# MILVLG/mmnas

Hardware: AMD Instinct MI355X
Metric: supernet fwd+bwd steps/sec (VQA arch, bs=64) (higher is better)
Workload: dtype f32 (bf16x6 split-operand MFMA, fp32 accumulate); 1 GPU; Net_Search supernet WEIGHT step: sample + fwd + BCE(sum) + bwd (+ gradient all-reduce), HSIZE 256, B=64/GPU, 100x2048 regions + 14 tokens, dropout 0.1 (search_vqa.py:279-292; BASELINE configs[2]); global_batch=64, parallelism=dp1, grad_allreduce=none, rccl_ranks=1, rank_id_sum_ok=True, lstm_fallback=False, dp_rows=1, dp_buckets=3, optimizer_in_step=False, gemm_split=6, hip_force_dev_kernarg=1

## Files before the change

### include/mmnas_hip.h

```cpp
#ifndef MMNAS_HIP_H
#define MMNAS_HIP_H

#include <stddef.h>
#include <stdint.h>

#ifdef __cplusplus
extern "C" {
#endif

#define MMNAS_ABI_VERSION 1

enum {
  MMNAS_OK = 0,
  MMNAS_E_SHAPE = -1,
  MMNAS_E_ARG = -2,
  MMNAS_E_LAUNCH = -3
};

enum {
  MMNAS_F_NORM = 1,
  MMNAS_F_RESIDUAL = 2,
  MMNAS_F_MASK = 4,
  MMNAS_F_REL = 8,
  MMNAS_F_SELF = 16,
// ... 146 lines not shown
int mmnas_rel_fused_bwd(const float* raw, const float* Wy, const float* by, const float* Wr,
                        const float* br, const float* dbiasT, float* dWy, float* dby, float* dWr,
                        float* dbr, float* ws, int B, int Sq, int Sk, int C, int R, int H,
                        void* stream);
int mmnas_rel_fused_fwd_ragged(const float* raw, const float* Wy, const float* by, const float* Wr, const float* br,
                               float* biasT, int B, int S, int C, int R, int H, const int* off, void* stream);
int mmnas_rel_fused_bwd_ragged(const float* raw, const float* Wy, const float* by, const float* Wr, const float* br,
                               const float* dbiasT, float* dWy, float* dby, float* dWr, float* dbr, float* ws,
                               int B, int S, int C, int R, int H, const int* off, const int* tile_off, int ntiles, void* stream);

#define MMNAS_REL_MULTI_MAX 32
typedef struct mmnas_rel_multi {
  int B, S, C, R, H, n_ops;
  const float* raw;
  const float* Wy; const float* by;
  float* dWy; float* dby;
  const float* Wr[MMNAS_REL_MULTI_MAX];
  const float* br[MMNAS_REL_MULTI_MAX];
  float* biasT[MMNAS_REL_MULTI_MAX];
  const float* dbiasT[MMNAS_REL_MULTI_MAX];
  float* dWr[MMNAS_REL_MULTI_MAX]; float* dbr[MMNAS_REL_MULTI_MAX];
  const int* off; const int* tile_off; int ntiles, reserved;
  float* ws;
} mmnas_rel_multi;
int mmnas_rel_multi_supported(int C, int R, int H);
size_t mmnas_rel_multi_bwd_ws_floats(int B, int S);
int mmnas_rel_multi_fwd(const mmnas_rel_multi* m, void* stream);
int mmnas_rel_multi_bwd(const mmnas_rel_multi* m, void* stream);
int mmnas_set_rel_hoist(int on);
int mmnas_set_guided_hoist(int on);
int mmnas_set_rel_overlap(int on);

typedef struct mmnas_mha_desc {
  int B, H, Sq, Sk, dh;
  int ldq, ldk, ldv, ldo;
  const float* Q; const float* K; const float* V;
  const uint8_t* mask;
  const float* biasT;
  float* O;
  float* lse;
  float drop_p; uint32_t drop_site; uint64_t drop_seed;
  const float* dO;
  float* dQ; float* dK; float* dV;
  float* dbiasT;
  float* delta;
  const int* q_off; const int* k_off;
} mmnas_mha_desc;

int mmnas_mha_core_fwd(const mmnas_mha_desc* d, void* stream);
int mmnas_mha_core_bwd(const mmnas_mha_desc* d, void* stream);
int mmnas_mha_core_fwd_indexed(const mmnas_mha_desc* d, const int* kv_idx, void* stream);

// ... 196 lines not shown
```

### mmnas_amd/_lib.py

```python
import ctypes as C
import logging
import os

import torch

from . import switches

_HERE = os.path.dirname(os.path.abspath(__file__))
LIB_PATH = os.environ.get(switches.LIB_PATH.name) or os.path.join(_HERE, 'lib', 'libmmnas_hip.so')

log = logging.getLogger('mmnas_amd')


def _launch_configuration():
    name = 'HIP_FORCE_DEV_KERNARG'
    if name in os.environ:
        return os.environ[name], 'inherited'
    if torch.cuda.is_initialized():
        log.warning('mmnas_amd was imported after HIP had initialised and %s is not set: kernel arguments go through host-visible '
                    'memory, the ~300 short launches of a step run 20-40 %% slower.  Export %s=1 or import mmnas / mmnas_amd '
                    'before the first CUDA call.', name, name)
        return None, 'unset_after_hip_init'
    os.environ[name] = '1'
    return '1', 'set_by_library'
# ... 75 lines not shown


class AttFlatSide(C.Structure):
    _fields_ = [('S', C.c_int), ('reserved', C.c_int), ('x', _fp), ('mask', _fp), ('W1', _fp), ('b1', _fp), ('W2', _fp),
                ('b2', _fp), ('Wm', _fp), ('bm', _fp), ('dW1', _fp), ('db1', _fp), ('dW2', _fp), ('db2', _fp), ('dWm', _fp),
                ('dbm', _fp), ('seed', C.c_uint64), ('dx', _fp), ('off', _fp), ('M', C.c_int), ('reserved2', C.c_int)]


class Head(C.Structure):
    _fields_ = [('B', C.c_int), ('d', C.c_int), ('MID', C.c_int), ('G', C.c_int), ('OUT', C.c_int), ('ANS', C.c_int),
                ('flags', C.c_int), ('reserved', C.c_int), ('drop_p', C.c_float), ('eps', C.c_float),
                ('sx', AttFlatSide), ('sy', AttFlatSide), ('ln_a', _fp), ('ln_b', _fp), ('dln_a', _fp), ('dln_b', _fp),
                ('Wp', _fp), ('bp', _fp), ('dWp', _fp), ('dbp', _fp), ('logits', _fp), ('dlogits', _fp), ('arena', _fp)]


REL_MULTI_MAX = 32


class RelMulti(C.Structure):
    _fields_ = [('B', C.c_int), ('S', C.c_int), ('C', C.c_int), ('R', C.c_int), ('H', C.c_int), ('n_ops', C.c_int),
                ('raw', _fp), ('Wy', _fp), ('by', _fp), ('dWy', _fp), ('dby', _fp),
                ('Wr', _fp * REL_MULTI_MAX), ('br', _fp * REL_MULTI_MAX), ('biasT', _fp * REL_MULTI_MAX),
                ('dbiasT', _fp * REL_MULTI_MAX), ('dWr', _fp * REL_MULTI_MAX), ('dbr', _fp * REL_MULTI_MAX),
                ('off', _fp), ('tile_off', _fp), ('ntiles', C.c_int), ('reserved', C.c_int), ('ws', _fp)]


class ProfStat(C.Structure):
    _fields_ = [('ms', C.c_double), ('flops', C.c_double), ('bytes', C.c_double), ('launches', C.c_long)]


K_NAMES = ['gemm', 'mha_fwd', 'mha_bwd', 'rel_fwd', 'rel_bwd', 'rowops', 'lstm', 'small_ops']


class Segment(C.Structure):
    _fields_ = [('ptr', _fp), ('offset', C.c_uint64), ('n', C.c_uint64)]


_i, _f, _u32, _u64, _sz = C.c_int, C.c_float, C.c_uint32, C.c_uint64, C.c_size_t
SYMBOLS = {
    'mmnas_abi_version': (_i, []),
    'mmnas_last_error': (C.c_char_p, []),
    'mmnas_switch_count': (_i, []),
    'mmnas_switch_info': (_i, [_i, C.POINTER(C.c_char_p), C.POINTER(C.c_char_p)] + [C.POINTER(_i)] * 3),
    'mmnas_dropout_mask': (_i, [_fp, _sz, _f, _u64, _u32, _fp]),
    'mmnas_gemm': (_i, [C.POINTER(GemmDesc), _fp]),
    'mmnas_split_planes': (_i, [_fp, _fp, _sz, _fp]),
    'mmnas_gemm_ln': (_i, [C.POINTER(GemmDesc), _fp, _fp, _fp, _f, _fp]),
# ... 34 lines not shown
    'mmnas_onehot_rows': (_i, [_fp, _i, _i, C.POINTER(C.c_int), _fp]),
    'mmnas_mixed_sum_ws_floats': (_sz, []),
    'mmnas_mixed_sum_fwd': (_i, [C.POINTER(_fp), _i, _fp, _fp, _sz, _fp]),
    'mmnas_mixed_sum_bwd': (_i, [C.POINTER(_fp), _i, _fp, _fp, _fp, _i, _fp, _fp, _sz, _fp]),
    'mmnas_alpha_full_step': (_i, [_fp, _fp, _fp, _fp, _fp, _i, _i, _f, _f, _f, _f, _i, _fp]),
    'mmnas_alpha_full_step_wd': (_i, [_fp, _fp, _fp, _fp, _fp, _i, _i, _f, _f, _f, _f, _f, _i, _fp]),
    'mmnas_alpha_two_step': (_i, [_fp, _fp, _fp, _fp, _fp, _i, _i, C.POINTER(C.c_int), _f, _f, _f, _f, _f, _i, _fp]),
    'mmnas_embedding_bwd': (_i, [_fp, _fp, _fp, C.c_long, _i, C.c_long, _fp]),
    'mmnas_node_mix_fwd': (_i, [_fp, _fp, _fp, _i, _fp, _fp, _i, _i, _f, _fp]),
    'mmnas_node_mix_bwd': (_i, [_fp, _fp, _fp, _i, _fp, _fp, _fp, _i, _fp, _fp, _i, _i, _f, _fp]),
    'mmnas_embedding_bwd_det': (_i, [_fp, _fp, _fp, _fp, C.c_long, _i, C.c_long, _f, _fp]),
    'mmnas_embedding_bwd_det_ws_floats': (_sz, [C.c_long, _i]),
    'mmnas_rel_fused_supported': (_i, [_i, _i, _i]),
    'mmnas_rel_fused_fwd': (_i, [_fp, _fp, _fp, _fp, _fp, _fp, _i, _i, _i, _i, _i, _i, _fp]),
    'mmnas_rel_fused_bwd_ws_floats': (_sz, [_i, _i, _i]),
    'mmnas_rel_fused_bwd': (_i, [_fp, _fp, _fp, _fp, _fp, _fp, _fp, _fp, _fp, _fp, _fp, _i, _i, _i, _i, _i, _i, _fp]),
    'mmnas_rel_fused_fwd_ragged': (_i, [_fp, _fp, _fp, _fp, _fp, _fp, _i, _i, _i, _i, _i, _fp, _fp]),
    'mmnas_rel_fused_bwd_ragged': (_i, [_fp] * 11 + [_i, _i, _i, _i, _i, _fp, _fp, _i, _fp]),
    'mmnas_rel_multi_supported': (_i, [_i, _i, _i]),
    'mmnas_rel_multi_bwd_ws_floats': (_sz, [_i, _i]),
    'mmnas_rel_multi_fwd': (_i, [C.POINTER(RelMulti), _fp]),
    'mmnas_rel_multi_bwd': (_i, [C.POINTER(RelMulti), _fp]),
    'mmnas_set_rel_hoist': (_i, [_i]),
    'mmnas_set_guided_hoist': (_i, [_i]),
    'mmnas_set_rel_overlap': (_i, [_i]),
    'mmnas_mha_core_fwd': (_i, [C.POINTER(MhaDesc), _fp]),
    'mmnas_mha_core_bwd': (_i, [C.POINTER(MhaDesc), _fp]),
    'mmnas_mha_core_fwd_indexed': (_i, [C.POINTER(MhaDesc), _fp, _fp]),
    'mmnas_itm_pair_head': (_i, [_fp] * 11 + [C.c_long, _i, _i, _f, _fp]),
    'mmnas_rank_matrix': (_i, [_fp, _i, _i, C.c_long, _fp, _fp, _fp, _fp, _fp, _fp]),
    'mmnas_row_topk': (_i, [_fp, _i, _i, C.c_long, _i, _fp, _fp, _fp]),
    'mmnas_vgd_targets': (_i, [_fp, _fp, _fp, _i, _i, C.c_double, _i, _fp, _fp, _fp, _fp, _fp, _fp, _fp]),
    'mmnas_vgd_ground': (_i, [_fp] * 5 + [_i, _i, C.c_double] + [_fp] * 7),
    'mmnas_vqa_answer': (_i, [_fp, _i, _i, C.c_long, _fp, C.c_long, _i, _i] + [_fp] * 4 + [_i] + [_fp] * 5),
    'mmnas_vqa_accuracy': (_i, [_fp] * 4 + [_i] * 4 + [_fp, _fp, _fp]),
    'mmnas_vqa_answer_targets': (_i, [_fp, _i, _i, _i, _fp, _fp, _fp]),
    'mmnas_vgd_loss_fwd': (_i, [_fp] * 6 + [_i] * 6 + [C.c_double, C.c_double] + [_fp] * 5),
    'mmnas_itm_triplet_loss_fwd': (_i, [_fp, _fp, _fp, C.c_long, _i, _f, _i, _fp, _fp, _fp]),
    'mmnas_loss_grad_scale': (_i, [_fp, _fp, _fp, _sz, _fp]),
    'mmnas_vgd_head_supported': (_i, [_i, _i]),
    'mmnas_vgd_head_bwd_ws_floats': (_sz, [_i, _i, _i]),
    'mmnas_vgd_head_fwd': (_i, [_fp] * 12 + [_i, _i, _i, _f, _i, _fp]),
    'mmnas_vgd_head_bwd': (_i, [_fp] * 20 + [_i, _i, _i, _f, _i, _fp]),
    'mmnas_att_op_plan': (_i, [C.POINTER(AttOp), C.POINTER(Plan)]),
    'mmnas_att_op_fwd': (_i, [C.POINTER(AttOp), _fp]),
    'mmnas_att_op_bwd': (_i, [C.POINTER(AttOp), _fp]),
# ... 78 lines not shown
```

### mmnas_amd/csrc/ops.hip

```cpp
#include <string.h>
#include <functional>
#include <vector>
#include "common.h"

namespace mmnas {

static inline size_t al(size_t n) { return (n + 255) & ~(size_t)255; }

struct Carver {
  char* base; size_t off;
  explicit Carver(void* p) : base((char*)p), off(0) {}
  float* take(size_t nfloats) { float* r = (float*)(base + off); off += al(nfloats * sizeof(float)); return r; }
};

static void gemm_init(mmnas_gemm_desc& g, int layout, int N, int K, int lda, int ldb, int ldc) {
  memset(&g, 0, sizeof(g));
  g.layout = layout; g.ngroups = 1; g.nseg = 1; g.N = N; g.K = K; g.lda = lda; g.ldb = ldb; g.ldc = ldc;
  g.alpha = 1.f; g.gate_scale = 1.f; g.split_k = 1;
}

struct AttLayout {
  size_t Mq, Mk;
  float *Q, *K, *V, *att, *stats, *z, *biasT;
  float *dz, *dt, *datt, *dQ, *dK, *dV, *delta, *dbiasT, *lnws, *relws;
// ... 712 lines not shown

static bool rel_hoist_on() { return sw::rel_hoist.get() != 0; }
struct RelGroups {
  std::vector<mmnas_rel_multi> groups[2];
  bool hoisted[MMNAS_CHAIN_MAX_OPS];
  RelGroups() { memset(hoisted, 0, sizeof(hoisted)); }
};
static void chain_rel_groups(const mmnas_chain* c, const ChainLayout& L, bool bwd, RelGroups& G) {
  if (!rel_hoist_on() || c->use_side_stream) return;
  char* base = (char*)c->arena;
  for (int i = 0; i < c->n_ops; ++i) {
    const mmnas_chain_op& o = c->ops[i];
    if (o.kind != MMNAS_CHAIN_ATT) continue;
    if (bwd && c->mixed && o.detached) continue;
    mmnas_att_op a; mmnas_mlp_op m;
    chain_op_setup(c, i, a, m);
    if (!(a.flags & MMNAS_F_REL) || !(a.flags & MMNAS_F_RELRAW) || !(a.flags & MMNAS_F_SELF)) continue;
    if (!mmnas_rel_multi_supported(a.C, a.R, a.H) || !a.rel || !a.Wy || !a.by) continue;
    if ((long)a.B * a.H * a.Sq * a.Sq >= (1l << 31)) continue;
    a.save = base + L.save[i]; a.ws = base + L.ws[i];
    const AttLayout al_ = att_layout(&a);
    std::vector<mmnas_rel_multi>& gs = G.groups[o.on_y ? 1 : 0];
    mmnas_rel_multi* g = nullptr;
    for (auto& q : gs)
      if (q.raw == a.rel && q.Wy == a.Wy && q.by == a.by && q.H == a.H && q.C == a.C && q.n_ops < MMNAS_REL_MULTI_MAX) { g = &q; break; }
    if (!g) {
      mmnas_rel_multi q;
      memset(&q, 0, sizeof(q));
      q.B = a.B; q.S = a.Sq; q.C = a.C; q.R = a.R; q.H = a.H;
      q.raw = a.rel; q.Wy = a.Wy; q.by = a.by; q.dWy = a.dWy; q.dby = a.dby;
      q.off = a.q_off; q.tile_off = a.rel_tile_off; q.ntiles = a.rel_ntiles;
      q.ws = (float*)(base + L.relws);
      gs.push_back(q);
      g = &gs.back();
    }
    const int j = g->n_ops++;
    g->Wr[j] = a.Wr; g->br[j] = a.br; g->biasT[j] = al_.biasT; g->dbiasT[j] = al_.dbiasT; g->dWr[j] = a.dWr; g->dbr[j] = a.dbr;
    G.hoisted[i] = true;
  }
}
static int chain_rel_fwd(const RelGroups& G, hipStream_t st, int only = -1) {
  for (int s = 0; s < 2; ++s)
    if (only < 0 || only == s)
      for (const auto& g : G.groups[s]) { const int rc = mmnas_rel_multi_fwd(&g, st); if (rc) return rc; }
  return MMNAS_OK;
}
static bool rel_overlap_on() { return sw::rel_overlap.get() != 0; }
static int chain_rel_bwd(const RelGroups& G, int stream_y, hipStream_t st) {
  for (const auto& g : G.groups[stream_y]) {
    MMNAS_REQUIRE(g.dWy && g.dby, MMNAS_E_ARG, "chain_bwd: relation operators without the stem layer's gradient sinks");
    const int rc = mmnas_rel_multi_bwd(&g, st);
    if (rc) return rc;
  }
  return MMNAS_OK;
// ... 820 lines not shown
```

### mmnas_amd/csrc/relmulti.hip

```cpp
#include <stdlib.h>
#include <string.h>
#include "common.h"

#ifndef MMNAS_DBG_REL
#define MMNAS_DBG_REL 0
#endif
#define RM_DBG(bit) (MMNAS_DBG_REL && (p.dbg & (bit)))

namespace mmnas {

constexpr int RM_R = 64;
constexpr int RM_CP = 8;
constexpr int RM_ROWS = 32;
constexpr int RM_NT_MAX = 3;
constexpr int RM_LDH = RM_R + 4;
constexpr int RM_LDP = RM_ROWS + 4;
constexpr int RM_ROW = RM_ROWS * RM_R + RM_R * RM_CP + RM_ROWS;

struct RelMultiK {
  const float* raw;
  int B, S, C, H, nrows, nops;
  int dbg;
  const int* off; const int* toff;
  float* part;
  const float* Wr[MMNAS_REL_MULTI_MAX];
  const float* br[MMNAS_REL_MULTI_MAX];
  float* io[RM_NT_MAX * RM_ROWS];
};

__device__ __forceinline__ void rm_locate(const RelMultiK& p, int T, int ntiles, int& b, int& tb) {
  if (T >= ntiles) { b = p.B; tb = 0; return; }
  int lo = 0, hi = p.B;
  while (hi - lo > 1) {
    const int mid = (lo + hi) >> 1;
    if (p.toff[mid] <= T) lo = mid; else hi = mid;
  }
  b = lo; tb = T - p.toff[lo];
}

struct RmWalk {
  int tile, ntiles, nwaves, tpb, cb, ct, adv_b, adv_t;
  __device__ __forceinline__ void init(const RelMultiK& p, int ntiles_, int tpb_, int w) {
    ntiles = ntiles_; tpb = tpb_;
    nwaves = (int)gridDim.x * 4;
    adv_b = nwaves / tpb; adv_t = nwaves - adv_b * tpb;
    tile = (int)blockIdx.x * 4 + w;
    cb = tile / tpb; ct = tile - cb * tpb;
    if (p.toff) rm_locate(p, tile, ntiles, cb, ct);
  }
  __device__ __forceinline__ void next(const RelMultiK& p) {
    tile += nwaves;
    cb += adv_b; ct += adv_t;
    if (ct >= tpb) { ct -= tpb; ++cb; }
    if (p.toff) rm_locate(p, tile, ntiles, cb, ct);
  }
};

struct RmElem { bool ok; int b; unsigned k, q, fc; };

__device__ __forceinline__ RmElem rm_elem(const RelMultiK& p, int b, int tb, int l31) {
  RmElem e;
  const unsigned S = (unsigned)p.S, SS = S * S;
  const unsigned f = (unsigned)tb * 32u + (unsigned)l31;
  bool ok = b < p.B && f < SS;
  unsigned wq = S;
  if (p.off) {
    const int bb = b < p.B ? b : 0;
    const int n = p.off[bb + 1] - p.off[bb];
    ok = b < p.B && n > 0 && f < (unsigned)n * (unsigned)n;
    wq = (unsigned)max(n, 1);
  }
  const unsigned f0 = ok ? f : 0u;
  e.ok = ok; e.b = ok ? b : 0;
  e.k = f0 / wq; e.q = f0 - e.k * wq;
  e.fc = e.k * S + e.q;
  return e;
}

typedef float f32x8 __attribute__((ext_vector_type(8)));
template <int C>
__device__ __forceinline__ f32x8 rm_raw(const RelMultiK& p, const RmElem& e) {
  const float* src = p.raw + (((size_t)e.b * p.S + e.q) * p.S + e.k) * C;
  f32x8 ex = {0.f, 0.f, 0.f, 0.f, 0.f, 0.f, 0.f, 0.f};
#pragma unroll
  for (int c = 0; c < C; ++c) { const float v = src[c]; ex[c] = e.ok ? v : 0.f; }
  ex[C] = e.ok ? 1.f : 0.f;
  return ex;
// ... 29 lines not shown

template <int C>
__device__ __forceinline__ void rm_wy_operand(const float* __restrict__ Wy, const float* __restrict__ by, int l31, int hh, float (*wyA)[4]) {
#pragma unroll
  for (int t = 0; t < 2; ++t)
#pragma unroll
    for (int s4 = 0; s4 < 4; ++s4) {
      const int j = 32 * t + l31, c = 2 * s4 + hh;
      wyA[t][s4] = c < C ? Wy[j * C + c] : (c == C ? by[j] : 0.f);
    }
}

template <int Y> __device__ __forceinline__ void rm_yield() {
  if constexpr (Y == 1) asm volatile("s_nop 1");
  if constexpr (Y == 3) asm volatile("s_nop 3");
}

template <int C, int NT, int Y>
__global__ void __launch_bounds__(256) rel_multi_fwd_kernel(const RelMultiK p, int ntiles, int tpb, const float* __restrict__ Wy,
                                                            const float* __restrict__ by) {
  __shared__ float sWrA[NT * RM_ROWS * RM_R];
  __shared__ __attribute__((aligned(16))) float sBr[NT * RM_ROWS];
  __shared__ __attribute__((aligned(16))) float* sIo[NT * RM_ROWS];
  const int tid = threadIdx.x, lane = tid & 63, w = tid >> 6, l31 = lane & 31, hh = lane >> 5;
  rm_stage_weights<false>(p, NT, sWrA, nullptr, sBr, sIo);
  float wyA[2][4];
  rm_wy_operand<C>(Wy, by, l31, hh, wyA);
  const unsigned SS = (unsigned)p.S * (unsigned)p.S;
  RmWalk wk;
  wk.init(p, ntiles, tpb, w);
  RmElem cur = rm_elem(p, wk.cb, wk.ct, l31);
  f32x8 ext = rm_raw<C>(p, cur);
  while (wk.tile < ntiles) {
    f32x16 hid[2];
#pragma unroll
    for (int t = 0; t < 2; ++t) {
#pragma unroll
      for (int r = 0; r < 16; ++r) hid[t][r] = 0.f;
#pragma unroll
      for (int s4 = 0; s4 < 4; ++s4) hid[t] = mfma32(wyA[t][s4], hh ? ext[2 * s4 + 1] : ext[2 * s4], hid[t]);
#pragma unroll
      for (int r = 0; r < 16; ++r) hid[t][r] = fmaxf(hid[t][r], 0.f);
    }
    const bool ok = cur.ok;
    const unsigned eoff = (unsigned)cur.b * (unsigned)p.H * SS + cur.fc;
    wk.next(p);
    cur = rm_elem(p, wk.cb, wk.ct, l31);
    if (!RM_DBG(2)) ext = rm_raw<C>(p, cur);
#pragma unroll
    for (int rt = 0; rt < NT; ++rt) {
      if (rt * RM_ROWS >= p.nrows) break;
      f32x16 rr;
#pragma unroll
      for (int r = 0; r < 16; ++r) rr[r] = 0.f;
#pragma unroll
      for (int t = 0; t < 2; ++t)
#pragma unroll
        for (int r = 0; r < 16; ++r) { if (!RM_DBG(4) || r == 0) { rr = mfma32(sWrA[(rt * 32 + 16 * t + r) * 64 + lane], hid[t][r], rr); rm_yield<Y>(); } }
#pragma unroll
      for (int u = 0; u < 4; ++u) {
        const int row = rt * RM_ROWS + 8 * u + 4 * hh;
        const float4 bq = *reinterpret_cast<const float4*>(sBr + row);
        const float bv[4] = {bq.x, bq.y, bq.z, bq.w};
#pragma unroll
        for (int i = 0; i < 4; ++i) {
          float* const o = sIo[row + i];
          if (ok && o && !(RM_DBG(1) && rr[4 * u + i] != 12345.f)) o[eoff] = __logf(fmaxf(rr[4 * u + i] + bv[i], 1e-6f));
        }
      }
    }
  }
}

template <int C, int Y>
__global__ void __launch_bounds__(256, 2) rel_multi_bwd_kernel(const RelMultiK p, int ntiles, int tpb, const float* __restrict__ Wy,
                                                               const float* __restrict__ by) {
  __shared__ __attribute__((aligned(16))) float sHidAll[4][32 * RM_LDH];
  __shared__ __attribute__((aligned(16))) float sDpreAll[4][32 * RM_LDP];
  __shared__ __attribute__((aligned(16))) float sRawAll[4][32 * RM_CP];
  __shared__ float sWrA[RM_ROWS * RM_R];
  __shared__ float sWrB[RM_ROWS * RM_R];
  __shared__ __attribute__((aligned(16))) float sBr[RM_ROWS];
  __shared__ __attribute__((aligned(16))) float* sIo[RM_ROWS];
  const int tid = threadIdx.x, lane = tid & 63, w = tid >> 6, l31 = lane & 31, hh = lane >> 5;
  const int l15 = lane & 15, q4 = lane >> 4;
  float* sHid = sHidAll[w];
  float* sDpre = sDpreAll[w];
  float* sRaw = sRawAll[w];
  rm_stage_weights<true>(p, 1, sWrA, sWrB, sBr, sIo);
  float wyA[2][4];
  rm_wy_operand<C>(Wy, by, l31, hh, wyA);

  f32x16 accWr[2];
  f32x4 accWy16[4];
  float accbr = 0.f;
#pragma unroll
  for (int r = 0; r < 16; ++r) { accWr[0][r] = 0.f; accWr[1][r] = 0.f; }
#pragma unroll
  for (int n = 0; n < 4; ++n)
#pragma unroll
    for (int r = 0; r < 4; ++r) accWy16[n][r] = 0.f;

  const unsigned SS = (unsigned)p.S * (unsigned)p.S;
  auto load_db = [&](const RmElem& e, float* db) __attribute__((always_inline)) {
    const unsigned eoff = (unsigned)e.b * (unsigned)p.H * SS + e.fc;
#pragma unroll
    for (int u = 0; u < 4; ++u)
#pragma unroll
      for (int i = 0; i < 4; ++i) {
        const float* const d = sIo[8 * u + 4 * hh + i];
        const bool live = e.ok && d != nullptr;
        const float v = (live ? d : p.raw)[live ? eoff : 0u];
        db[4 * u + i] = live ? v : 0.f;
      }
  };
  RmWalk wk;
  wk.init(p, ntiles, tpb, w);
  RmElem cur = rm_elem(p, wk.cb, wk.ct, l31);
  float db[16];
  f32x8 ext = rm_raw<C>(p, cur);
  load_db(cur, db);
  while (wk.tile < ntiles) {
    f32x16 hid[2];
    unsigned gm = 0u;
#pragma unroll
    for (int t = 0; t < 2; ++t) {
#pragma unroll
      for (int r = 0; r < 16; ++r) hid[t][r] = 0.f;
#pragma unroll
      for (int s4 = 0; s4 < 4; ++s4) hid[t] = mfma32(wyA[t][s4], hh ? ext[2 * s4 + 1] : ext[2 * s4], hid[t]);
#pragma unroll
      for (int r = 0; r < 16; ++r) {
        gm |= hid[t][r] > 0.f ? (1u << (16 * t + r)) : 0u;
        hid[t][r] = fmaxf(hid[t][r], 0.f);
      }
    }
    f32x16 rr;
#pragma unroll
    for (int r = 0; r < 16; ++r) rr[r] = 0.f;
#pragma unroll
    for (int t = 0; t < 2; ++t)
// ... 4 lines not shown
    for (int u = 0; u < 4; ++u) {
      const float4 bq = *reinterpret_cast<const float4*>(sBr + 8 * u + 4 * hh);
      const float bv[4] = {bq.x, bq.y, bq.z, bq.w};
#pragma unroll
      for (int i = 0; i < 4; ++i) {
        const float rv = rr[4 * u + i] + bv[i];
        dpre[4 * u + i] = rv >= 1e-6f ? db[4 * u + i] / rv : 0.f;
      }
    }
    asm volatile("s_waitcnt lgkmcnt(0)" ::: "memory");
#pragma unroll
    for (int t = 0; t < 2; ++t)
#pragma unroll
      for (int u = 0; u < 4; ++u)
        *reinterpret_cast<float4*>(sHid + l31 * RM_LDH + 32 * t + 8 * u + 4 * hh) =
            make_float4(hid[t][4 * u], hid[t][4 * u + 1], hid[t][4 * u + 2], hid[t][4 * u + 3]);
#pragma unroll
    for (int u = 0; u < 4; ++u)
      *reinterpret_cast<float4*>(sDpre + l31 * RM_LDP + 8 * u + 4 * hh) = make_float4(dpre[4 * u], dpre[4 * u + 1], dpre[4 * u + 2], dpre[4 * u + 3]);
    if (hh == 0) {
      *reinterpret_cast<float4*>(sRaw + l31 * RM_CP) = make_float4(ext[0], ext[1], ext[2], ext[3]);
      *reinterpret_cast<float4*>(sRaw + l31 * RM_CP + 4) = make_float4(ext[4], ext[5], ext[6], ext[7]);
    }
    wk.next(p);
    cur = rm_elem(p, wk.cb, wk.ct, l31);
    ext = rm_raw<C>(p, cur);
    load_db(cur, db);
    f32x16 dh[2];
#pragma unroll
    for (int t = 0; t < 2; ++t) {
#pragma unroll
      for (int r = 0; r < 16; ++r) dh[t][r] = 0.f;
#pragma unroll
      for (int r = 0; r < 16; ++r) { dh[t] = mfma32(sWrB[(16 * t + r) * 64 + lane], dpre[r], dh[t]); rm_yield<Y>(); }
#pragma unroll
      for (int r = 0; r < 16; ++r) dh[t][r] = (gm >> (16 * t + r)) & 1u ? dh[t][r] : 0.f;
    }
    asm volatile("s_waitcnt lgkmcnt(0)" ::: "memory");
#pragma unroll
    for (int s0 = 0; s0 < 16; s0 += 4) {
      float av[4], b0[4], b1[4];
#pragma unroll
      for (int u = 0; u < 4; ++u) {
        const int e = 2 * (s0 + u) + hh;
        av[u] = sDpre[e * RM_LDP + l31];
        b0[u] = sHid[e * RM_LDH + l31];
        b1[u] = sHid[e * RM_LDH + 32 + l31];
      }
// ... 108 lines not shown
    const int o = col - RM_ROWS * RM_R, j = o / RM_CP, c = o - j * RM_CP;
    if (c < p.C) p.dWy[j * p.C + c] += v;
    else if (c == p.C) p.dby[j] += v;
  } else {
    const int row = col - RM_ROWS * RM_R - RM_R * RM_CP;
    if (row < p.nrows) { const int n = row / p.H, h = row - n * p.H; p.dbr[n][h] += v; }
  }
}

static int rm_check(const mmnas_rel_multi* m, const char* who) {
  MMNAS_REQUIRE(m, MMNAS_E_ARG, "%s: null descriptor", who);
  MMNAS_REQUIRE(m->B > 0 && m->S > 0, MMNAS_E_SHAPE, "%s: B=%d S=%d", who, m->B, m->S);
  MMNAS_REQUIRE(m->R == RM_R, MMNAS_E_SHAPE, "%s: REL_SIZE=%d (the fused path handles 64)", who, m->R);
  MMNAS_REQUIRE(m->C == 3 || m->C == 4, MMNAS_E_SHAPE, "%s: %d raw relation channels (3 or 4)", who, m->C);
  MMNAS_REQUIRE(m->H >= 1 && m->H <= RM_ROWS && RM_ROWS % m->H == 0, MMNAS_E_SHAPE, "%s: H=%d heads (a divisor of 32)", who, m->H);
  MMNAS_REQUIRE(m->n_ops >= 1 && m->n_ops <= MMNAS_REL_MULTI_MAX, MMNAS_E_SHAPE, "%s: %d operators (1..%d)", who, m->n_ops, MMNAS_REL_MULTI_MAX);
  MMNAS_REQUIRE(m->raw && m->Wy && m->by, MMNAS_E_ARG, "%s: null pointer", who);
  MMNAS_REQUIRE((long)m->B * m->H * m->S * m->S < (1l << 31), MMNAS_E_SHAPE, "%s: B H S^2 must fit 31 bits", who);
  if (m->off) MMNAS_REQUIRE(m->tile_off && m->ntiles >= 0, MMNAS_E_ARG, "%s: ragged batches need the tile offsets", who);
  return MMNAS_OK;
}

static long rm_tiles_per_b(int S) { return ((long)S * S + 31) / 32; }
static int rm_grid(long ntiles, int per_cu) {
  const long wgs = (ntiles + 3) / 4, cap = 256l * per_cu;
  return (int)(wgs < 1 ? 1 : (wgs < cap ? wgs : cap));
}

}

using namespace mmnas;

extern "C" int mmnas_rel_multi_supported(int C, int R, int H) { return R == RM_R && (C == 3 || C == 4) && H >= 1 && H <= RM_ROWS && RM_ROWS % H == 0; }

extern "C" size_t mmnas_rel_multi_bwd_ws_floats(int B, int S) {
  return (size_t)rm_grid((long)B * rm_tiles_per_b(S), 2) * RM_ROW;
}

extern "C" int mmnas_rel_multi_fwd(const mmnas_rel_multi* m, void* stream) {
  int rc = rm_check(m, "rel_multi_fwd");
  if (rc) return rc;
  hipStream_t st = (hipStream_t)stream;
  const int tpb = (int)rm_tiles_per_b(m->S);
  const int ntiles = m->off ? m->ntiles : m->B * tpb;
  if (ntiles == 0) return MMNAS_OK;
  const int ops_per_tile = RM_ROWS / m->H;
  const int max_ops = ops_per_tile * RM_NT_MAX;
  const unsigned SS = (unsigned)m->S * (unsigned)m->S;
  for (int o0 = 0; o0 < m->n_ops; o0 += max_ops) {
    const int n = m->n_ops - o0 < max_ops ? m->n_ops - o0 : max_ops;
    RelMultiK k;
    memset(&k, 0, sizeof(k));
    k.raw = m->raw; k.B = m->B; k.S = m->S; k.C = m->C; k.H = m->H; k.off = m->off; k.toff = m->tile_off;
    k.dbg = sw::rel_multi_dbg.get();
    for (int j = 0; j < n; ++j) {
      MMNAS_REQUIRE(m->Wr[o0 + j] && m->br[o0 + j] && m->biasT[o0 + j], MMNAS_E_ARG, "rel_multi_fwd: operator %d: null pointer", o0 + j);
      for (int h = 0; h < m->H; ++h) k.io[j * m->H + h] = m->biasT[o0 + j] + (size_t)h * SS;
    }
    const int slots = n * m->H;
    for (int j = 0; j < n; ++j) { k.Wr[j] = m->Wr[o0 + j]; k.br[j] = m->br[o0 + j]; }
    k.nops = n; k.nrows = slots;
    const int nt = (slots + RM_ROWS - 1) / RM_ROWS;
    const int fwd_per_cu = sw::rel_multi_wgs.get();
    const int grid = rm_grid(ntiles, fwd_per_cu);
    const double ne = m->off ? 32.0 * ntiles : (double)m->B * SS;
    ProfScope ps(MMNAS_K_REL_FWD, 2.0 * ne * (RM_R * (m->C + 1) + (double)n * m->H * RM_R), 4.0 * ne * (m->C + n * m->H), st);
    const int yield = sw::rel_multi_yield.get();
#define RM_FWD(CC, NTT) do { if (yield == 1) MMNAS_LAUNCH((rel_multi_fwd_kernel<CC, NTT, 1>), dim3(grid), dim3(256), 0, st, k, ntiles, tpb, m->Wy, m->by); \
      else if (yield == 3) MMNAS_LAUNCH((rel_multi_fwd_kernel<CC, NTT, 3>), dim3(grid), dim3(256), 0, st, k, ntiles, tpb, m->Wy, m->by); \
      else MMNAS_LAUNCH((rel_multi_fwd_kernel<CC, NTT, 0>), dim3(grid), dim3(256), 0, st, k, ntiles, tpb, m->Wy, m->by); } while (0)
    if (m->C == 4) { if (nt == 1) RM_FWD(4, 1); else if (nt == 2) RM_FWD(4, 2); else RM_FWD(4, 3); }
    else { if (nt == 1) RM_FWD(3, 1); else if (nt == 2) RM_FWD(3, 2); else RM_FWD(3, 3); }
#undef RM_FWD
    if ((rc = check_launch("rel_multi_fwd"))) return rc;
  }
  return MMNAS_OK;
}

extern "C" int mmnas_rel_multi_bwd(const mmnas_rel_multi* m, void* stream) {
  int rc = rm_check(m, "rel_multi_bwd");
  if (rc) return rc;
  MMNAS_REQUIRE(m->dWy && m->dby && m->ws, MMNAS_E_ARG, "rel_multi_bwd: null pointer");
  hipStream_t st = (hipStream_t)stream;
  const int tpb = (int)rm_tiles_per_b(m->S);
  const int ntiles = m->off ? m->ntiles : m->B * tpb;
  if (ntiles == 0) return MMNAS_OK;
  const int max_ops = RM_ROWS / m->H;
  const unsigned SS = (unsigned)m->S * (unsigned)m->S;
  for (int o0 = 0; o0 < m->n_ops; o0 += max_ops) {
    const int n = m->n_ops - o0 < max_ops ? m->n_ops - o0 : max_ops;
    RelMultiK k;
    RelMultiRed red;
    memset(&k, 0, sizeof(k));
    memset(&red, 0, sizeof(red));
    k.raw = m->raw; k.B = m->B; k.S = m->S; k.C = m->C; k.H = m->H; k.off = m->off; k.toff = m->tile_off;
    k.part = m->ws; k.nops = n; k.nrows = n * m->H;
    for (int j = 0; j < n; ++j) {
      MMNAS_REQUIRE(m->Wr[o0 + j] && m->br[o0 + j] && m->dbiasT[o0 + j] && m->dWr[o0 + j] && m->dbr[o0 + j], MMNAS_E_ARG,
                    "rel_multi_bwd: operator %d: null pointer", o0 + j);
      k.Wr[j] = m->Wr[o0 + j]; k.br[j] = m->br[o0 + j];
      red.dWr[j] = m->dWr[o0 + j]; red.dbr[j] = m->dbr[o0 + j];
      for (int h = 0; h < m->H; ++h) k.io[j * m->H + h] = const_cast<float*>(m->dbiasT[o0 + j]) + (size_t)h * SS;
    }
    const int grid = rm_grid(ntiles, 2);
    red.part = m->ws; red.nrows_part = grid; red.C = m->C; red.H = m->H; red.nrows = k.nrows; red.dWy = m->dWy; red.dby = m->dby;
    const double ne = m->off ? 32.0 * ntiles : (double)m->B * SS;
    const double rows = (double)n * m->H;
    ProfScope ps(MMNAS_K_REL_BWD, 2.0 * ne * (2.0 * RM_R * (m->C + 1) + 3.0 * rows * RM_R), 4.0 * ne * (m->C + rows), st);
    const int yield = sw::rel_multi_yield.get();
#define RM_BWD(CC) do { if (yield == 1) MMNAS_LAUNCH((rel_multi_bwd_kernel<CC, 1>), dim3(grid), dim3(256), 0, st, k, ntiles, tpb, m->Wy, m->by); \
      else if (yield == 3) MMNAS_LAUNCH((rel_multi_bwd_kernel<CC, 3>), dim3(grid), dim3(256), 0, st, k, ntiles, tpb, m->Wy, m->by); \
      else MMNAS_LAUNCH((rel_multi_bwd_kernel<CC, 0>), dim3(grid), dim3(256), 0, st, k, ntiles, tpb, m->Wy, m->by); } while (0)
    if (m->C == 4) RM_BWD(4); else RM_BWD(3);
#undef RM_BWD
    MMNAS_LAUNCH(rel_multi_reduce_kernel, dim3(cdiv(RM_ROW, 64)), dim3(1024), 0, st, red);
    if ((rc = check_launch("rel_multi_bwd"))) return rc;
  }
  return MMNAS_OK;
// ... 2 lines not shown
```

### mmnas_amd/csrc/switches.h

```cpp
#pragma once

namespace mmnas {

int env_int(const char* name, int dflt);

enum SwKind { sw_int, sw_bool, sw_exact1, sw_presence, sw_string };
enum SwPolicy { sw_once, sw_every_call, sw_reload };

struct Switch {
  const char* name;
  int dflt;
  SwKind kind;
  SwPolicy policy;
  const char* help;
  int value;
  int state;

  int get() { return state ? value : read(); }
  int read();
  int reload();
  int set(int v);
  int peek(int* source) const;
};

// ... 9 lines not shown
  X(guided_hoist, "MMNAS_GUIDED_HOIST", 1, bool, once, "key / value projections of a chain's guided operators as grouped launches (mmnas_set_guided_hoist)") \
  X(rel_fwd_valu, "MMNAS_REL_FWD_VALU", 0, exact1, every_call, "1: a lone RelSelfAtt computes its bias with the per-operator fused kernel instead of the one-operator multi kernel (A/B)") \
  X(side_prio, "MMNAS_SIDE_PRIO", 1, bool, every_call, "0: the chains' extra streams without stream priorities (read when a stream pair is created)") \
  X(side_flush, "MMNAS_SIDE_FLUSH", 0, string, once, "op: side-stream parameter-gradient work released behind every operator instead of once per phase") \
   \
  X(small_ops, "MMNAS_SMALL_OPS", 1, bool, once, "SelfAtt of <= 16 rows as one launch forward (mmnas_set_small_ops); 0: the general path") \
  X(small_bwd, "MMNAS_SMALL_BWD", 1, bool, once, "the same operators' backward as two launches (mmnas_set_small_bwd)") \
  X(small_ffn, "MMNAS_SMALL_FFN", 0, int, once, "FeedForward forward as one launch (mmnas_set_small_ffn): 1 four slices of 256 hidden units, 2 eight of 128; measured neutral (profiles/r05_small_ffn_ab.txt)") \
   \
  X(gemm_ln, "MMNAS_GEMM_LN", 0, exact1, once, "1: the merge / last FFN product and its LayerNorm as one row-panel launch (mmnas_set_gemm_ln); measured neutral, profiles/r06_ab.txt") \
  X(gemm_ln_minm, "MMNAS_GEMM_LN_MINM", 2048, int, once, "fewest rows for the row-panel kernel (read together with MMNAS_GEMM_LN)") \
  X(gemm_ln_maxk, "MMNAS_GEMM_LN_MAXK", 256, int, once, "largest K for the row-panel kernel (read together with MMNAS_GEMM_LN)") \
   \
  X(mha_nw, "MMNAS_MHA_NW", 4, int, every_call, "2: attention cores never use 4-wave workgroups (4-wave groups measured 7-15 % faster)") \
  X(mha_pair, "MMNAS_MHA_PAIR", 1, bool, once, "0: two attention cores of one geometry as two launches (mixed chain)") \
  X(mha_bwd_fused, "MMNAS_MHA_BWD_FUSED", 1, bool, once, "0: the attention backward as separate dQ and dK / dV kernels (dense rows only)") \
  X(mha_fwd_b16, "MMNAS_MHA_FWD_B16", 1, bool, once, "0: attention forward (d_h = 64, 65..128 keys) on the fp32 MFMA kernels instead of split-bf16 operands (profiles/r06_attention_b16_ab.txt)") \
  X(mha_fwd_b16_two, "MMNAS_MHA_FWD_B16_TWO", 320, int, once, "more than this many (sample, head) pairs: the split-bf16 forward runs two per workgroup") \
  X(mha_bwd_b16, "MMNAS_MHA_BWD_B16", 1, bool, once, "0: attention backward (d_h = 64, 65..128 keys) on the fp32 MFMA kernels instead of split-bf16 operands (supernet step -1.6 % with both)") \
   \
  X(rel_multi_dbg, "MMNAS_REL_MULTI_DBG", 0, int, once, "timing experiments of a -DMMNAS_DBG_REL=1 build only (wrong results): 1 no stores, 2 no raw reloads, 4 no head-projection MFMAs") \
  X(rel_multi_wgs, "MMNAS_REL_MULTI_WGS", 3, int, once, "workgroups per CU of the multi-operator relation forward (tuning)") \
  X(rel_multi_yield, "MMNAS_REL_MULTI_YIELD", 0, int, once, "1 | 3: the multi-operator relation kernels' yield variants (tuning)") \
  X(rel_bwd_valu, "MMNAS_REL_BWD_VALU", 1, bool, once, "0: the fused relation backward as the all-MFMA kernel (A/B)") \
   \
  X(gemm_tile, "MMNAS_GEMM_TILE", 0, int, reload, "64 | 128: force the tile shape") \
  X(gemm_generic, "MMNAS_GEMM_GENERIC", 0, presence, reload, "set (to anything): force the guarded-load path; ops.py reads it too") \
  X(gemm_sk, "MMNAS_GEMM_SK", 1, int, reload, "stream-K / split-K: 0 never, 1 automatic, 2 always") \
  X(gemm_wgs, "MMNAS_GEMM_WGS", 0, int, reload, "co-resident workgroup budget (0: 1024 for 64^2 tiles, 512 for 128^2)") \
  X(gemm_min_units, "MMNAS_GEMM_MIN_UNITS", 4, int, reload, "fewest K-tiles a workgroup is given (at least 1)") \
  X(gemm_gm, "MMNAS_GEMM_GM", 0, int, reload, "row-panels per tile-order block (0: 8)") \
  X(gemm_xcd, "MMNAS_GEMM_XCD", 1, int, reload, "0: identity workgroup mapping") \
  X(gemm_split, "MMNAS_GEMM_SPLIT", 6, int, reload, "products as 6 / 3 / 1 bf16 MFMA products of split operands (6: fp32-grade; 3, 1: reduced precision), 0: fp32 MFMA") \
  X(gemm_pair, "MMNAS_GEMM_PAIR", 1, int, reload, "0: mmnas_gemm_pair launches its two products separately") \
  X(gemm_split_slots, "MMNAS_GEMM_SPLIT_SLOTS", 0, int, reload, "split-K pieces wanted over all tiles (0: from SPLIT_P and SPLIT_MINWG)") \
  X(gemm_split_p, "MMNAS_GEMM_SPLIT_P", 24, int, reload, "K-tiles per split-K piece (at least 1)") \
  X(gemm_split_minwg, "MMNAS_GEMM_SPLIT_MINWG", 256, int, reload, "fewest split-K pieces in total when pieces of SPLIT_P would be fewer") \
  X(gemm_pf, "MMNAS_GEMM_PF", 2, int, reload, "1 | 2: K-tiles of operand loads in flight ahead of the MFMA block (64^2 fp32 path)") \
  X(gemm_hyb_t, "MMNAS_GEMM_HYB_T", 16, int, reload, "fewest K-tiles per output tile for the whole-tiles + streamed-tail hybrid") \
  X(gemm_wide_min, "MMNAS_GEMM_WIDE_MIN", 200, int, reload, "fewest 128x64 tiles for that shape to be chosen") \
  X(gemm_lean, "MMNAS_GEMM_LEAN", 3, int, reload, "lean kernels: bit 0 NT / NN products, bit 1 split-K TN products") \
  X(gemm_lean_maxb, "MMNAS_GEMM_LEAN_MAXB", 8 << 20, int, reload, "largest B matrix (bytes) the lean tile order is used for") \
  X(lstm_fwd_p, "MMNAS_LSTM_FWD_P", 0, int, every_call, "K-tiles per workgroup of the LSTM forward step's stream-K product (0: whole tiles; read per time step)") \
  X(lstm_bwd_p, "MMNAS_LSTM_BWD_P", 8, int, every_call, "K-tiles per workgroup of the LSTM backward step's stream-K product (0: whole tiles; read per time step)") \
   \
  X(prof_dump, "MMNAS_PROF_DUMP", 0, string, every_call, "file: mmnas_prof_collect appends one kind,tag,ms,flops,bytes row per bracketed launch (tools/prof_shapes.py)")
// ... 9 lines not shown
```

Measured before the change: 225.0 steps/s.

## Limit relation multi-op kernels to elements under each sample's last unmasked key

The multi-operator relation forward and backward kernels now take the key padding mask. Each workgroup scans it to find every sample's last unmasked key and builds a per-sample tile table in shared memory. Tiles are then walked only over the unmasked prefix of S*S elements instead of all of them, which cuts work on padded region batches. In exchange, every workgroup pays for a redundant mask scan and prefix sum. Elements past the limit are no longer written, which relies on downstream consumers masking them.

Result: faster. 227.8 steps/s (median of 6 runs) (+1.3%).

```diff
diff --git a/include/mmnas_hip.h b/include/mmnas_hip.h
--- a/include/mmnas_hip.h
+++ b/include/mmnas_hip.h
@@ -192,12 +192,14 @@
   float* dWr[MMNAS_REL_MULTI_MAX]; float* dbr[MMNAS_REL_MULTI_MAX];
   const int* off; const int* tile_off; int ntiles, reserved;
   float* ws;
+  const unsigned char* key_mask;
 } mmnas_rel_multi;
 int mmnas_rel_multi_supported(int C, int R, int H);
 size_t mmnas_rel_multi_bwd_ws_floats(int B, int S);
 int mmnas_rel_multi_fwd(const mmnas_rel_multi* m, void* stream);
 int mmnas_rel_multi_bwd(const mmnas_rel_multi* m, void* stream);
 int mmnas_set_rel_hoist(int on);
+int mmnas_set_rel_keylimit(int on);
 int mmnas_set_guided_hoist(int on);
 int mmnas_set_rel_overlap(int on);
 
diff --git a/mmnas_amd/_lib.py b/mmnas_amd/_lib.py
--- a/mmnas_amd/_lib.py
+++ b/mmnas_amd/_lib.py
@@ -121,7 +121,7 @@
                 ('raw', _fp), ('Wy', _fp), ('by', _fp), ('dWy', _fp), ('dby', _fp),
                 ('Wr', _fp * REL_MULTI_MAX), ('br', _fp * REL_MULTI_MAX), ('biasT', _fp * REL_MULTI_MAX),
                 ('dbiasT', _fp * REL_MULTI_MAX), ('dWr', _fp * REL_MULTI_MAX), ('dbr', _fp * REL_MULTI_MAX),
-                ('off', _fp), ('tile_off', _fp), ('ntiles', C.c_int), ('reserved', C.c_int), ('ws', _fp)]
+                ('off', _fp), ('tile_off', _fp), ('ntiles', C.c_int), ('reserved', C.c_int), ('ws', _fp), ('key_mask', _fp)]
 
 
 class ProfStat(C.Structure):
@@ -202,6 +202,7 @@
     'mmnas_rel_multi_fwd': (_i, [C.POINTER(RelMulti), _fp]),
     'mmnas_rel_multi_bwd': (_i, [C.POINTER(RelMulti), _fp]),
     'mmnas_set_rel_hoist': (_i, [_i]),
+    'mmnas_set_rel_keylimit': (_i, [_i]),
     'mmnas_set_guided_hoist': (_i, [_i]),
     'mmnas_set_rel_overlap': (_i, [_i]),
     'mmnas_mha_core_fwd': (_i, [C.POINTER(MhaDesc), _fp]),
diff --git a/mmnas_amd/csrc/ops.hip b/mmnas_amd/csrc/ops.hip
--- a/mmnas_amd/csrc/ops.hip
+++ b/mmnas_amd/csrc/ops.hip
@@ -758,14 +758,16 @@
     const AttLayout al_ = att_layout(&a);
     std::vector<mmnas_rel_multi>& gs = G.groups[o.on_y ? 1 : 0];
     mmnas_rel_multi* g = nullptr;
+    const unsigned char* const kmask = (a.flags & MMNAS_F_MASK) ? (const unsigned char*)a.mask : nullptr;
     for (auto& q : gs)
-      if (q.raw == a.rel && q.Wy == a.Wy && q.by == a.by && q.H == a.H && q.C == a.C && q.n_ops < MMNAS_REL_MULTI_MAX) { g = &q; break; }
+      if (q.raw == a.rel && q.Wy == a.Wy && q.by == a.by && q.H == a.H && q.C == a.C && q.key_mask == kmask && q.n_ops < MMNAS_REL_MULTI_MAX) { g = &q; break; }
     if (!g) {
       mmnas_rel_multi q;
       memset(&q, 0, sizeof(q));
       q.B = a.B; q.S = a.Sq; q.C = a.C; q.R = a.R; q.H = a.H;
       q.raw = a.rel; q.Wy = a.Wy; q.by = a.by; q.dWy = a.dWy; q.dby = a.dby;
       q.off = a.q_off; q.tile_off = a.rel_tile_off; q.ntiles = a.rel_ntiles;
+      q.key_mask = kmask;
       q.ws = (float*)(base + L.relws);
       gs.push_back(q);
       g = &gs.back();
diff --git a/mmnas_amd/csrc/relmulti.hip b/mmnas_amd/csrc/relmulti.hip
--- a/mmnas_amd/csrc/relmulti.hip
+++ b/mmnas_amd/csrc/relmulti.hip
@@ -15,6 +15,7 @@
 constexpr int RM_NT_MAX = 3;
 constexpr int RM_LDH = RM_R + 4;
 constexpr int RM_LDP = RM_ROWS + 4;
+constexpr int RM_KB_MAX = 256;
 constexpr int RM_ROW = RM_ROWS * RM_R + RM_R * RM_CP + RM_ROWS;
 
 struct RelMultiK {
@@ -22,47 +23,91 @@
   int B, S, C, H, nrows, nops;
   int dbg;
   const int* off; const int* toff;
+  const unsigned char* kmask;
   float* part;
   const float* Wr[MMNAS_REL_MULTI_MAX];
   const float* br[MMNAS_REL_MULTI_MAX];
   float* io[RM_NT_MAX * RM_ROWS];
 };
 
-__device__ __forceinline__ void rm_locate(const RelMultiK& p, int T, int ntiles, int& b, int& tb) {
-  if (T >= ntiles) { b = p.B; tb = 0; return; }
-  int lo = 0, hi = p.B;
+__device__ __forceinline__ void rm_key_table(const RelMultiK& p, unsigned* lim, int* toff) {
+  const int tid = threadIdx.x, B = p.B, S = p.S;
+  int tps = 64;
+  while (tps > 1 && tps * B > 256) tps >>= 1;
+  const int b = tid / tps, c = tid - b * tps;
+  int last = 0;
+  if (b < B) {
+    const unsigned char* __restrict__ row = p.kmask + (size_t)b * S;
+    if ((((size_t)p.kmask | (size_t)S) & 3) == 0) {
+      const unsigned* __restrict__ row4 = reinterpret_cast<const unsigned*>(row);
+#pragma unroll 8
+      for (int j = c; j < (S >> 2); j += tps) {
+        const unsigned v = row4[j];
+        const int hi = !(v >> 24) ? 4 : !(v & 0xff0000u) ? 3 : !(v & 0xff00u) ? 2 : !(v & 0xffu) ? 1 : 0;
+        last = hi ? 4 * j + hi : last;
+      }
+    } else {
+#pragma unroll 8
+      for (int k = c; k < S; k += tps) last = row[k] ? last : k + 1;
+    }
+  }
+  for (int d = 1; d < tps; d <<= 1) last = max(last, __shfl_xor(last, d, 64));
+  if (b < B && c == 0) lim[b] = (unsigned)last * (unsigned)S;
+  __syncthreads();
+  if (tid < 64) {
+    int t[4], s = 0;
+#pragma unroll
+    for (int i = 0; i < 4; ++i) { const int bb = 4 * tid + i; t[i] = bb < B ? (int)((lim[bb] + 31u) >> 5) : 0; s += t[i]; }
+    int run = s;
+    for (int d = 1; d < 64; d <<= 1) { const int o = __shfl_up(run, d, 64); if (tid >= d) run += o; }
+    run -= s;
+#pragma unroll
+    for (int i = 0; i < 4; ++i) { const int bb = 4 * tid + i; run += t[i]; if (bb < B) toff[bb + 1] = run; }
+    if (tid == 0) toff[0] = 0;
+  }
+  __syncthreads();
+}
+
+__device__ __forceinline__ void rm_locate(const int* toff, int B, int T, int ntiles, int& b, int& tb) {
+  if (T >= ntiles) { b = B; tb = 0; return; }
+  int lo = 0, hi = B;
   while (hi - lo > 1) {
     const int mid = (lo + hi) >> 1;
-    if (p.toff[mid] <= T) lo = mid; else hi = mid;
-  }
-  b = lo; tb = T - p.toff[lo];
+    if (toff[mid] <= T) lo = mid; else hi = mid;
+  }
+  b = lo; tb = T - toff[lo];
 }
 
 struct RmWalk {
   int tile, ntiles, nwaves, tpb, cb, ct, adv_b, adv_t;
-  __device__ __forceinline__ void init(const RelMultiK& p, int ntiles_, int tpb_, int w) {
+  __device__ __forceinline__ void locate(const RelMultiK& p, const int* ktoff) {
+    if (p.kmask) rm_locate(ktoff, p.B, tile, ntiles, cb, ct);
+    else if (p.toff) rm_locate(p.toff, p.B, tile, ntiles, cb, ct);
+  }
+  __device__ __forceinline__ void init(const RelMultiK& p, const int* ktoff, int ntiles_, int tpb_, int w) {
     ntiles = ntiles_; tpb = tpb_;
     nwaves = (int)gridDim.x * 4;
     adv_b = nwaves / tpb; adv_t = nwaves - adv_b * tpb;
     tile = (int)blockIdx.x * 4 + w;
     cb = tile / tpb; ct = tile - cb * tpb;
-    if (p.toff) rm_locate(p, tile, ntiles, cb, ct);
-  }
-  __device__ __forceinline__ void next(const RelMultiK& p) {
+    locate(p, ktoff);
+  }
+  __device__ __forceinline__ void next(const RelMultiK& p, const int* ktoff) {
     tile += nwaves;
     cb += adv_b; ct += adv_t;
     if (ct >= tpb) { ct -= tpb; ++cb; }
-    if (p.toff) rm_locate(p, tile, ntiles, cb, ct);
+    locate(p, ktoff);
   }
 };
 
 struct RmElem { bool ok; int b; unsigned k, q, fc; };
 
-__device__ __forceinline__ RmElem rm_elem(const RelMultiK& p, int b, int tb, int l31) {
+__device__ __forceinline__ RmElem rm_elem(const RelMultiK& p, const unsigned* klim, int b, int tb, int l31) {
   RmElem e;
   const unsigned S = (unsigned)p.S, SS = S * S;
   const unsigned f = (unsigned)tb * 32u + (unsigned)l31;
   bool ok = b < p.B && f < SS;
+  if (p.kmask) ok = b < p.B && f < klim[b < p.B ? b : 0];
   unsigned wq = S;
   if (p.off) {
     const int bb = b < p.B ? b : 0;
@@ -138,14 +183,17 @@
   __shared__ float sWrA[NT * RM_ROWS * RM_R];
   __shared__ __attribute__((aligned(16))) float sBr[NT * RM_ROWS];
   __shared__ __attribute__((aligned(16))) float* sIo[NT * RM_ROWS];
+  __shared__ unsigned sKlim[RM_KB_MAX];
+  __shared__ int sKtoff[RM_KB_MAX + 1];
   const int tid = threadIdx.x, lane = tid & 63, w = tid >> 6, l31 = lane & 31, hh = lane >> 5;
+  if (p.kmask) { rm_key_table(p, sKlim, sKtoff); ntiles = sKtoff[p.B]; }
   rm_stage_weights<false>(p, NT, sWrA, nullptr, sBr, sIo);
   float wyA[2][4];
   rm_wy_operand<C>(Wy, by, l31, hh, wyA);
   const unsigned SS = (unsigned)p.S * (unsigned)p.S;
   RmWalk wk;
-  wk.init(p, ntiles, tpb, w);
-  RmElem cur = rm_elem(p, wk.cb, wk.ct, l31);
+  wk.init(p, sKtoff, ntiles, tpb, w);
+  RmElem cur = rm_elem(p, sKlim, wk.cb, wk.ct, l31);
   f32x8 ext = rm_raw<C>(p, cur);
   while (wk.tile < ntiles) {
     f32x16 hid[2];
@@ -160,8 +208,8 @@
     }
     const bool ok = cur.ok;
     const unsigned eoff = (unsigned)cur.b * (unsigned)p.H * SS + cur.fc;
-    wk.next(p);
-    cur = rm_elem(p, wk.cb, wk.ct, l31);
+    wk.next(p, sKtoff);
+    cur = rm_elem(p, sKlim, wk.cb, wk.ct, l31);
     if (!RM_DBG(2)) ext = rm_raw<C>(p, cur);
 #pragma unroll
     for (int rt = 0; rt < NT; ++rt) {
@@ -198,8 +246,11 @@
   __shared__ float sWrB[RM_ROWS * RM_R];
   __shared__ __attribute__((aligned(16))) float sBr[RM_ROWS];
   __shared__ __attribute__((aligned(16))) float* sIo[RM_ROWS];
+  __shared__ unsigned sKlim[RM_KB_MAX];
+  __shared__ int sKtoff[RM_KB_MAX + 1];
   const int tid = threadIdx.x, lane = tid & 63, w = tid >> 6, l31 = lane & 31, hh = lane >> 5;
   const int l15 = lane & 15, q4 = lane >> 4;
+  if (p.kmask) { rm_key_table(p, sKlim, sKtoff); ntiles = sKtoff[p.B]; }
   float* sHid = sHidAll[w];
   float* sDpre = sDpreAll[w];
   float* sRaw = sRawAll[w];
@@ -231,8 +282,8 @@
       }
   };
   RmWalk wk;
-  wk.init(p, ntiles, tpb, w);
-  RmElem cur = rm_elem(p, wk.cb, wk.ct, l31);
+  wk.init(p, sKtoff, ntiles, tpb, w);
+  RmElem cur = rm_elem(p, sKlim, wk.cb, wk.ct, l31);
   float db[16];
   f32x8 ext = rm_raw<C>(p, cur);
   load_db(cur, db);
@@ -283,8 +334,8 @@
       *reinterpret_cast<float4*>(sRaw + l31 * RM_CP) = make_float4(ext[0], ext[1], ext[2], ext[3]);
       *reinterpret_cast<float4*>(sRaw + l31 * RM_CP + 4) = make_float4(ext[4], ext[5], ext[6], ext[7]);
     }
-    wk.next(p);
-    cur = rm_elem(p, wk.cb, wk.ct, l31);
+    wk.next(p, sKtoff);
+    cur = rm_elem(p, sKlim, wk.cb, wk.ct, l31);
     ext = rm_raw<C>(p, cur);
     load_db(cur, db);
     f32x16 dh[2];
@@ -439,6 +490,9 @@
 }
 
 static long rm_tiles_per_b(int S) { return ((long)S * S + 31) / 32; }
+static const unsigned char* rm_key_mask(const mmnas_rel_multi* m) {
+  return (m->key_mask && !m->off && m->B <= RM_KB_MAX && sw::rel_keylimit.get()) ? m->key_mask : nullptr;
+}
 static int rm_grid(long ntiles, int per_cu) {
   const long wgs = (ntiles + 3) / 4, cap = 256l * per_cu;
   return (int)(wgs < 1 ? 1 : (wgs < cap ? wgs : cap));
@@ -447,6 +501,8 @@
 }
 
 using namespace mmnas;
+
+extern "C" int mmnas_set_rel_keylimit(int on) { return sw::rel_keylimit.set(on != 0); }
 
 extern "C" int mmnas_rel_multi_supported(int C, int R, int H) { return R == RM_R && (C == 3 || C == 4) && H >= 1 && H <= RM_ROWS && RM_ROWS % H == 0; }
 
@@ -469,6 +525,7 @@
     RelMultiK k;
     memset(&k, 0, sizeof(k));
     k.raw = m->raw; k.B = m->B; k.S = m->S; k.C = m->C; k.H = m->H; k.off = m->off; k.toff = m->tile_off;
+    k.kmask = rm_key_mask(m);
     k.dbg = sw::rel_multi_dbg.get();
     for (int j = 0; j < n; ++j) {
       MMNAS_REQUIRE(m->Wr[o0 + j] && m->br[o0 + j] && m->biasT[o0 + j], MMNAS_E_ARG, "rel_multi_fwd: operator %d: null pointer", o0 + j);
@@ -511,6 +568,7 @@
     memset(&k, 0, sizeof(k));
     memset(&red, 0, sizeof(red));
     k.raw = m->raw; k.B = m->B; k.S = m->S; k.C = m->C; k.H = m->H; k.off = m->off; k.toff = m->tile_off;
+    k.kmask = rm_key_mask(m);
     k.part = m->ws; k.nops = n; k.nrows = n * m->H;
     for (int j = 0; j < n; ++j) {
       MMNAS_REQUIRE(m->Wr[o0 + j] && m->br[o0 + j] && m->dbiasT[o0 + j] && m->dWr[o0 + j] && m->dbr[o0 + j], MMNAS_E_ARG,
diff --git a/mmnas_amd/csrc/switches.h b/mmnas_amd/csrc/switches.h
--- a/mmnas_amd/csrc/switches.h
+++ b/mmnas_amd/csrc/switches.h
@@ -55,6 +55,7 @@
   X(rel_multi_dbg, "MMNAS_REL_MULTI_DBG", 0, int, once, "timing experiments of a -DMMNAS_DBG_REL=1 build only (wrong results): 1 no stores, 2 no raw reloads, 4 no head-projection MFMAs") \
   X(rel_multi_wgs, "MMNAS_REL_MULTI_WGS", 3, int, once, "workgroups per CU of the multi-operator relation forward (tuning)") \
   X(rel_multi_yield, "MMNAS_REL_MULTI_YIELD", 0, int, once, "1 | 3: the multi-operator relation kernels' yield variants (tuning)") \
+  X(rel_keylimit, "MMNAS_REL_KEYLIMIT", 1, int, once, "multi-operator relation kernels of a padded batch walk only the elements under keys up to each sample's last unmasked one (mmnas_set_rel_keylimit); 0: all B S^2 elements") \
   X(rel_bwd_valu, "MMNAS_REL_BWD_VALU", 1, bool, once, "0: the fused relation backward as the all-MFMA kernel (A/B)") \
    \
   X(gemm_tile, "MMNAS_GEMM_TILE", 0, int, reload, "64 | 128: force the tile shape") \
```
